# Youssef-Harby/flac-raster

Hardware: AMD Instinct MI355X
Metric: Mpixels/sec encode (create-streaming) + bbox-extract ms, 1/2/4/8 GPU; bit-exact vs ref (higher is better)
Workload: dtype int16; 1 GPU; C4 create-streaming encode (band 1, device-resident); raster=40000x40000x4 int16, tile_size=512, tiles=6241, tiles_rank0=6241, blocksize=4096, compression_level=5, parallelism=single GPU (no exchange), compressed_bytes_rank0=3134407161, compressed_bytes_total=3134407161

## Files before the change

### flac_raster_amd/csrc/frs_encode.hip

```cpp

#include <type_traits>

#include <cstring>
#include <unistd.h>

#include "frs_internal.h"
#include "frs_frame_header.h"
#include "frs_crc16_fold.h"

namespace frs {

template <int DT> struct Elem;
template <> struct Elem<FRS_DT_U8> { using T = uint8_t; static constexpr bool is_float = false; };
template <> struct Elem<FRS_DT_U16> { using T = uint16_t; static constexpr bool is_float = false; };
template <> struct Elem<FRS_DT_I16> { using T = int16_t; static constexpr bool is_float = false; };
template <> struct Elem<FRS_DT_I32> { using T = int32_t; static constexpr bool is_float = false; };
template <> struct Elem<FRS_DT_U32> { using T = uint32_t; static constexpr bool is_float = false; };
template <> struct Elem<FRS_DT_F32> { using T = float; static constexpr bool is_float = true; };
template <> struct Elem<FRS_DT_F64> { using T = double; static constexpr bool is_float = true; };

__device__ inline int64_t f2key(double v) {
    int64_t b = __double_as_longlong(v);
    return b >= 0 ? b : (b ^ 0x7FFFFFFFFFFFFFFFll);
}
// ... 2254 lines not shown
    v ^= bfly_partner<32>(v);
    return uni(v);
}
__device__ inline uint32_t dpp_incl_scan_u32(uint32_t v) {
    v += (uint32_t)__builtin_amdgcn_update_dpp(0, (int)v, 0x111, 0xF, 0xF, false);
    v += (uint32_t)__builtin_amdgcn_update_dpp(0, (int)v, 0x112, 0xF, 0xF, false);
    v += (uint32_t)__builtin_amdgcn_update_dpp(0, (int)v, 0x114, 0xF, 0xF, false);
    v += (uint32_t)__builtin_amdgcn_update_dpp(0, (int)v, 0x118, 0xF, 0xF, false);
    v += (uint32_t)__builtin_amdgcn_update_dpp(0, (int)v, 0x142, 0xA, 0xF, false);
    v += (uint32_t)__builtin_amdgcn_update_dpp(0, (int)v, 0x143, 0xC, 0xF, false);
    return v;
}
__device__ inline uint32_t dpp_wave_shr1(uint32_t v) {
    return (uint32_t)__builtin_amdgcn_update_dpp(0, (int)v, 0x138, 0xF, 0xF, false);
}

typedef short v2s16 __attribute__((ext_vector_type(2)));
__device__ inline int32_t dot2(uint32_t a, uint32_t b, int32_t c) {
    return __builtin_amdgcn_sdot2(__builtin_bit_cast(v2s16, a), __builtin_bit_cast(v2s16, b), c, false);
}
__device__ inline uint32_t pack2(int32_t lo, int32_t hi) { return ((uint32_t)lo & 0xFFFFu) | ((uint32_t)hi << 16); }

__device__ inline int32_t dot2_z(uint32_t a, uint32_t b) {
    int32_t d;
    asm("v_dot2_i32_i16 %0, %1, %2, 0" : "=v"(d) : "v"(a), "v"(b));
    return d;
}

__device__ inline void residual_pair(const uint32_t *E, const uint32_t *C, int shift, int m, int32_t &re, int32_t &ro) {
    const int b = 4 + m;
    const uint32_t o0 = __builtin_amdgcn_perm(E[b], E[b - 1], 0x05040302u);
    const uint32_t o1 = __builtin_amdgcn_perm(E[b - 1], E[b - 2], 0x05040302u);
    const uint32_t o2 = __builtin_amdgcn_perm(E[b - 2], E[b - 3], 0x05040302u);
    const uint32_t o3 = __builtin_amdgcn_perm(E[b - 3], E[b - 4], 0x05040302u);
    int32_t se = dot2_z(E[b - 1], C[0]);
    int32_t so = dot2_z(o0, C[0]);
    se = dot2(E[b - 2], C[1], se);
    so = dot2(o1, C[1], so);
    se = dot2(E[b - 3], C[2], se);
    so = dot2(o2, C[2], so);
    se = dot2(E[b - 4], C[3], se);
    so = dot2(o3, C[3], so);
    const uint32_t v = E[b];
    re = (int32_t)(int16_t)(v & 0xFFFFu) - (se >> shift);
    ro = ((int32_t)v >> 16) - (so >> shift);
}

constexpr uint64_t kFlagAgg = 1ull << 62, kFlagIncl = 2ull << 62, kValMask = (1ull << 62) - 1;


constexpr int kXpowHi = (kXpowBytes + 63) / 64;
constexpr int kBufWordsV3 = kFrameWordsV3 + 64;
constexpr int kSubWords = kFrameWordsV3 + 4;
struct EncV3Shared {
    uint32_t bits[4][kBufWordsV3];
    int16_t lut[kLutCap];
    uint16_t xlo[64];
    uint16_t xhi[kXpowHi + 3];
    uint8_t crc8[256];
    int ticket[2];
    int want[2];
    int lut_tile;
};
static_assert(offsetof(EncV3Shared, lut) + sizeof(int16_t) * kLutCap <= 65536, "LUT beyond 64 KiB of LDS");

struct FbMap {
    uint32_t c, magic, k;
    __device__ inline uint32_t col(uint32_t w) const { return __umul24(w, magic) >> 20; }
    __device__ inline uint32_t operator()(uint32_t w) const {
        return (uint32_t)__mul24((int)col(w), -(int)k) + (w << 6);
    }
};
__device__ inline FbMap fb_map(uint32_t words) {
    const uint32_t c = max(1u, (words + 63) >> 6);
    return FbMap{c, ((1u << 20) + c - 1) / c, 64 * c - 1};
}
__device__ inline void fb_fold(uint32_t *buf, const FbMap &M, int lane) {
    uint32_t *ovr = buf + (M.c << 6) + lane;
    const uint32_t v = *ovr;
    *ovr = 0;
    if (lane < 63 && v) atomicOr(buf + lane + 1, v);
}

__device__ inline void lds_put_bits2(uint32_t *buf, const FbMap &M, uint32_t pos, uint32_t val, int nbits) {
    const uint32_t wi = pos >> 5;
    const uint64_t v = (uint64_t)val << (64 - (int)(pos & 31) - nbits);
    atomicOr(&buf[M(wi)], (uint32_t)(v >> 32));
    atomicOr(&buf[M(wi + 1)], (uint32_t)v);
}

__device__ inline void reg_fence(uint32_t *E) {
#pragma unroll
    for (int m = 0; m < 36; m++) asm volatile("" : "+v"(E[m]));
}

__device__ inline uint32_t sad_u32(uint32_t a, uint32_t b, uint32_t c) {
    uint32_t d;
    asm("v_sad_u32 %0, %1, %2, %3" : "=v"(d) : "v"(a), "v"(b), "v"(c));
    return d;
}

__device__ inline void lds_put_left(uint32_t *buf, const FbMap &M, int nk4, uint32_t pos, uint32_t codeL) {
    const uint32_t hi = __builtin_amdgcn_alignbit(0u, codeL, pos);
    const uint32_t lo = __builtin_amdgcn_alignbit(codeL, 0u, pos);
    const uint32_t wi = pos >> 5;
    uint32_t *p = reinterpret_cast<uint32_t *>(reinterpret_cast<char *>(buf) + (wi << 8) +
                                               __mul24((int)M.col(wi), nk4));
    atomicOr(p, hi);
    atomicOr(p + 64, lo);
}

__device__ inline void lut_gather_pairs(const uint32_t *w, const int16_t *lut, int32_t imin, uint32_t *out) {
    const uint32_t lb = (uint32_t)reinterpret_cast<uintptr_t>(lut);
    const uint32_t c16 = (lb - 2u * (uint32_t)imin) & 0xFFFFu, cc = c16 | (c16 << 16), two = 0x00020002u;
    const char *lds0 = reinterpret_cast<const char *>(lut) - lb;
#pragma unroll
    for (int m = 0; m < 32; m++) {
        uint32_t a;
        asm("v_pk_mad_u16 %0, %1, %2, %3" : "=v"(a) : "v"(w[m]), "v"(two), "v"(cc));
        const uint32_t lo = *reinterpret_cast<const uint16_t *>(lds0 + (a & 0xFFFFu));
        const uint32_t hi = *reinterpret_cast<const uint16_t *>(lds0 + (a >> 16));
        out[m] = lo | (hi << 16);
    }
}

__device__ inline uint32_t zigzag(int32_t r) { return ((uint32_t)r << 1) ^ (uint32_t)(r >> 31); }

struct PendingFrame {
    int64_t f = -1;
    uint64_t fbytes = 0;
    bool ok = true;
    FbMap map{1, 1u << 20, 63};
};

__device__ __forceinline__ void resolve_and_store(const EncodeParams &P, PendingFrame &pf, uint32_t *fbuf, uint8_t *arena,
                                         int64_t arena_cap, int64_t *frame_off, uint64_t *status, int *err, int lane) {
    const int64_t f = pf.f;
    const uint64_t fbytes = pf.fbytes;
    const bool ok = pf.ok;
    const bool l0 = lane == 0;
    uint64_t prefix = 0;
    if (f > 0) {
        constexpr int kPer = 1;
        int64_t hi = f - 1;
        uint64_t accum = 0;
        long spins = 0;
// ... 2 lines not shown
#pragma unroll
            for (int i = 0; i < kPer; i++) {
                const int64_t j = hi - (int64_t)(lane * kPer + i);
                sv[i] = kFlagIncl;
                if (j >= 0) sv[i] = __hip_atomic_load(&status[j], __ATOMIC_RELAXED, __HIP_MEMORY_SCOPE_AGENT);
            }
            int my_first = kPer;
#pragma unroll
            for (int i = kPer - 1; i >= 0; i--)
                if ((sv[i] >> 62) == 2) my_first = i;
            const uint64_t has = __ballot(my_first < kPer);
            const int fl = has ? __builtin_ctzll(has) : 64;
            const int first_i = fl < 64 ? __builtin_amdgcn_readlane(my_first, fl) : kPer;
            bool missing = false;
            uint64_t mine = 0;
#pragma unroll
            for (int i = 0; i < kPer; i++) {
                const bool need = lane < fl || (lane == fl && i <= first_i);
                if (need) {
                    missing |= (sv[i] >> 62) == 0;
                    mine += sv[i] & kValMask;
                }
            }
            if (__ballot(missing)) {
                if (++spins > (1l << 22)) {
                    if (l0) atomicOr(err, 8);
                    break;
                }
                __builtin_amdgcn_s_setprio(0);
                if (spins < 4) __builtin_amdgcn_s_sleep(2);
                else if (spins < 16) __builtin_amdgcn_s_sleep(8);
                else __builtin_amdgcn_s_sleep(32);
                __builtin_amdgcn_s_setprio(2);
                continue;
            }
            accum += dpp_wave_sum_u64(mine);
            if (fl < 64) break;
            hi -= 64 * kPer;
        }
        prefix = accum;
    }
    if (l0) {
        if (f > 0)
            __hip_atomic_store(&status[f], kFlagIncl | (prefix + fbytes), __ATOMIC_RELAXED, __HIP_MEMORY_SCOPE_AGENT);
        frame_off[f] = (int64_t)prefix;
    }
    const FbMap M = pf.map;
    if ((int64_t)(prefix + fbytes) > arena_cap) {
        if (l0) atomicOr(err, 16);
    } else if (fbytes) {
        uint8_t *dst = arena + prefix;
        const uint32_t a0 = min((uint32_t)fbytes, (uint32_t)((16 - (reinterpret_cast<uintptr_t>(dst) & 15)) & 15));
        auto byte_at = [&](uint32_t b) -> uint8_t { return (uint8_t)(fbuf[M(b >> 2)] >> (24 - 8 * (b & 3))); };
        if ((uint32_t)lane < a0) dst[lane] = byte_at((uint32_t)lane);
        const uint32_t n16 = ((uint32_t)fbytes - a0) >> 4;
        const uint32_t r = a0 & 3, sb = a0 >> 2;
        uint4 *d16 = reinterpret_cast<uint4 *>(dst + a0);
        auto chunk = [&](uint32_t ci) {
            const uint32_t wq = sb + 4 * ci;
            const uint32_t w0 = __builtin_bswap32(fbuf[M(wq)]), w1 = __builtin_bswap32(fbuf[M(wq + 1)]);
            const uint32_t w2 = __builtin_bswap32(fbuf[M(wq + 2)]), w3 = __builtin_bswap32(fbuf[M(wq + 3)]);
            const uint32_t w4 = __builtin_bswap32(fbuf[M(wq + 4)]);
            uint4 o4;
            o4.x = __builtin_amdgcn_alignbyte(w1, w0, r);
            o4.y = __builtin_amdgcn_alignbyte(w2, w1, r);
            o4.z = __builtin_amdgcn_alignbyte(w3, w2, r);
            o4.w = __builtin_amdgcn_alignbyte(w4, w3, r);
            d16[ci] = o4;
        };
        const uint32_t c0 = (uint32_t)lane * M.c, c1 = c0 + M.c;
        const uint32_t ci0 = c0 > sb ? (c0 - sb + 3) >> 2 : 0u, ci1 = c1 > sb ? min(n16, (c1 - sb + 3) >> 2) : 0u;
        if (ci0 < ci1) {
            const uint32_t *cp = fbuf + M(sb + 4 * ci0);
            for (uint32_t ci = ci0; ci + 1 < ci1; ci++, cp += 256) {
                const uint32_t w0 = __builtin_bswap32(cp[0]), w1 = __builtin_bswap32(cp[64]);
                const uint32_t w2 = __builtin_bswap32(cp[128]), w3 = __builtin_bswap32(cp[192]);
                const uint32_t w4 = __builtin_bswap32(cp[256]);
                uint4 o4;
                o4.x = __builtin_amdgcn_alignbyte(w1, w0, r);
                o4.y = __builtin_amdgcn_alignbyte(w2, w1, r);
                o4.z = __builtin_amdgcn_alignbyte(w3, w2, r);
                o4.w = __builtin_amdgcn_alignbyte(w4, w3, r);
                d16[ci] = o4;
            }
            chunk(ci1 - 1);
        }
        const uint32_t tb = a0 + 16 * n16 + (uint32_t)lane;
        if (tb < (uint32_t)fbytes) dst[tb] = byte_at(tb);
    }
    if (ok) {
        for (uint32_t i = 0; i < M.c; i++) fbuf[(i << 6) | (uint32_t)lane] = 0;
    } else {
        for (uint32_t i = (uint32_t)lane; i < (uint32_t)kBufWordsV3; i += 64) fbuf[i] = 0;
    }
    pf.f = -1;
}

__device__ inline void fixed_lane_totals(const uint32_t *E, bool l0, uint32_t *tk, uint32_t *hk) {
    constexpr uint32_t M = 0x80000000u;
    const int32_t h1 = (int32_t)E[3] >> 16, h2 = (int16_t)(E[3] & 0xFFFFu);
    const int32_t h3 = (int32_t)E[2] >> 16, h4 = (int16_t)(E[2] & 0xFFFFu);
    uint32_t p0 = (uint32_t)h1 ^ M, p1 = (uint32_t)(h1 - h2) ^ M, p2 = (uint32_t)((h1 - h2) - (h2 - h3)) ^ M;
    uint32_t p3 = (uint32_t)(((h1 - h2) - (h2 - h3)) - ((h2 - h3) - (h3 - h4))) ^ M;
    uint32_t t0 = 0, t1 = 0, t2 = 0, t3 = 0, t4 = 0;
#pragma unroll
    for (int k = 0; k < 5; k++) hk[k] = 0;
#pragma unroll
// ... 252 lines not shown
            bb[c] = best_bits;
            bp[c] = 5 - best_i;
            bk[c] = (int)((Kp[c] >> (4 * best_i)) & 15u);
        }
    };
    auto rice = [&](uint32_t lane_sum, int order, uint32_t &best_bits, int &best_po, int &my_k) {
        if (__ballot(lane_sum >= (1u << 24)) == 0) {
            const uint32_t sm[1] = {lane_sum};
            const int od[1] = {order};
            uint32_t b1[1];
            int p1[1], k1[1];
            rice32m(std::integral_constant<int, 1>{}, sm, od, b1, p1, k1);
            best_bits = b1[0], best_po = p1[0], my_k = k1[0];
        } else {
            rice64(lane_sum, order, best_bits, best_po, my_k);
        }
    };
    rb_f = rb_l = 0;
    po_f = po_l = k_f = k_l = 0;
    if (cand_fixed && cand_lpc && __ballot(sf >= (1u << 24) || sl >= (1u << 24)) == 0) {
        uint32_t bb[2];
        int bp[2], bk[2];
        const uint32_t sm[2] = {sf, sl};
        const int od[2] = {of, ol};
        rice32m(std::integral_constant<int, 2>{}, sm, od, bb, bp, bk);
        rb_f = bb[0], po_f = bp[0], k_f = bk[0];
        rb_l = bb[1], po_l = bp[1], k_l = bk[1];
    } else {
        if (cand_fixed) rice(sf, of, rb_f, po_f, k_f);
        if (cand_lpc) rice(sl, ol, rb_l, po_l, k_l);
    }
}

constexpr int kPrivRows = 34;
constexpr uint32_t kPrivBits = kPrivRows * 32;
static_assert(kBufWordsV3 >= (kPrivRows + 1) * 64, "private rows + the spill row");
static_assert(kBufWordsV3 % 4 == 0, "b128 zeroing");

__device__ inline void zero_wave_buf(uint32_t *buf, int lane) {
    uint4 *b4 = reinterpret_cast<uint4 *>(buf);
#pragma unroll
    for (int i = 0; i < (kBufWordsV3 / 4 + 63) / 64; i++) {
        const int c = lane + 64 * i;
        if (i < kBufWordsV3 / 256 || c < kBufWordsV3 / 4) b4[c] = make_uint4(0u, 0u, 0u, 0u);
    }
}

constexpr int kCrcRows = kFrameWordsV3 / 64;
constexpr int kCrcBias = 192;
static_assert(kFrameWordsV3 % 64 == 0 && kCrcRows <= frs::kCrcFoldSpan && kCrcBias % 64 == 0 && kCrcBias >= 4 * kCrcRows,
              "column CRC");
static_assert(kCrcRows * 64 <= kBufWordsV3 && sizeof(g_xpow_hi) == sizeof(uint16_t) * (kXpowHi + 3),
              "the rows read (in groups of 8, below kCrcRows) are the buffer's; the factor table");
__device__ __forceinline__ uint32_t crc16_cols(const uint32_t *fbuf, const FbMap &M, uint32_t body, const EncV3Shared &S,
                                               int lane) {
    const uint32_t c = frs::crc16_column<kCrcRows, 8>(fbuf + lane, 64, (int)M.c);
    const int m = max(0, (int)body + (kCrcBias - 4 * kCrcRows) - 4 * (int)M.c * lane);
    return dpp_wave_xor_u32(gf_mulmod(gf_mulmod(c, S.xlo[m & 63]), S.xhi[m >> 6]));
}

template <int DT, bool SUB = false, bool ST = false, bool WIDE = false>
__device__ __forceinline__ void encode_frame_v4(const typename Elem<DT>::T *raster, const EncodeParams &P,
                                                const TileGeom *__restrict__ tiles,
                                                const TileNorm *__restrict__ norms,
                                                const SubAnalysis *__restrict__ ana, uint8_t *arena, int64_t arena_cap,
                                                int64_t *frame_off, uint64_t *status, int *err, EncV3Shared &S,
                                                int want, int64_t f, int lane, const int32_t *ftile,
                                                PendingFrame &prev, const uint4 *hdr_tab, int hdr_n,
                                                const uint32_t *pslots, const int64_t *pbytes, int chn = 0,
                                                uint32_t *sub_slots = nullptr, int32_t *sub_bits = nullptr,
                                                int32_t *sub_est = nullptr) {
    using T = typename Elem<DT>::T;
    using Lane = std::conditional_t<WIDE, LaneWide, LanePairs>;
    uint32_t *fbuf = S.bits[uni_if<!WIDE>(threadIdx.x >> 6)];
    const int t = ftile[f];
    const TileGeom g = tiles[t];
    const bool l0 = lane == 0;
    if (!SUB && g.partial && f - g.frame_base == g.nframes - 1) {
        const int64_t si = g.partial - 1;
        const uint64_t nb = (uint64_t)pbytes[si];
        const uint32_t words = (uint32_t)((nb + 3) >> 2);
        const bool ok = words + 2 <= (uint32_t)kFrameWordsV3;
        if (!ok && l0) atomicOr(err, 2);
        const uint64_t fbytes = ok ? nb : 0;
        const FbMap M = fb_map(words + 1);
        __builtin_amdgcn_s_setprio(2);
        if (l0)
            __hip_atomic_store(&status[f], (f == 0 ? kFlagIncl : kFlagAgg) | fbytes, __ATOMIC_RELAXED,
                               __HIP_MEMORY_SCOPE_AGENT);
        if (prev.f >= 0) resolve_and_store(P, prev, fbuf, arena, arena_cap, frame_off, status, err, lane);
        if (ok) {
            const uint32_t *src = pslots + (size_t)si * P.slot_words;
            for (uint32_t w = (uint32_t)lane; w < words; w += 64) fbuf[M(w)] = __builtin_bswap32(src[w]);
        }
        __builtin_amdgcn_s_waitcnt(0xC07F);
        __builtin_amdgcn_wave_barrier();
        __builtin_amdgcn_s_setprio(0);
        prev.f = f, prev.fbytes = fbytes, prev.ok = ok, prev.map = M;
        return;
    }
    TileNorm tn = norms[t];
    if (t != want && tn.mode == kNormLut) tn.mode = kNormSlow;
    const int16_t *lut = S.lut;
    __builtin_amdgcn_s_setprio(2);
    const int64_t fk = f - g.frame_base;
    const int64_t s0 = fk * kMaxBlock;
    constexpr int n = kMaxBlock;
    const int64_t sub = SUB ? f * P.nvch + chn : f;
    const SubAnalysis A = ana[sub];
    const int w = A.wasted;
    const int sbps = 16 - w + ((ST && chn == 3) ? 1 : 0);
    const T *base = raster + (int64_t)(P.band0 + ((ST && chn >= 2) ? 0 : chn)) * P.band_stride + g.r0 * P.row_stride +
                    g.c0;

    auto load_lane = [&](Lane &Ls) __attribute__((always_inline)) {
        Chunk64<DT> ch;
        const uint32_t sl0 = (uint32_t)s0 + 64u * (uint32_t)lane;
        const uint32_t row = udiv_inv(sl0, (uint32_t)g.w, 1.0 / (double)g.w);
        const int col = (int)(sl0 - row * (uint32_t)g.w), vec = (g.w % 64) == 0 ? P.vec_ok : 0;
// ... 334 lines not shown
        const int typecode = type == 0 ? 0 : type == 1 ? 1 : type == 2 ? 8 + of : 32 + ol - 1;
        lds_put_bits2(fbuf, M, hdr_bits, (uint32_t)(typecode << 1) | (w ? 1u : 0u), 8);
        if (w) lds_put_bits2(fbuf, M, hdr_bits + 8 + (uint32_t)(w - 1), 1, 1);
        if (type == 0) lds_put_bits2(fbuf, M, pos0, xi & ((1u << sbps) - 1u), sbps);
        if (type >= 2) {
            uint32_t qq = pos0 + (uint32_t)o * sbps;
            if (type == 3) {
                lds_put_bits2(fbuf, M, qq, (uint32_t)(A.lpc_prec - 1), 4);
                lds_put_bits2(fbuf, M, qq + 4, (uint32_t)lshift & 31u, 5);
                qq += 9 + (uint32_t)o * A.lpc_prec;
            }
            lds_put_bits2(fbuf, M, qq, (uint32_t)po, 6);
        }
    }
    if (type >= 2) {
        const int i = lane & 7;
        const int32_t qi = ana[sub].q[i];
        const bool warm = lane < 8 && i < o, coef = type == 3 && lane >= 8 && lane < 16 && i < o;
        if (warm) lds_put_bits2(fbuf, M, pos0 + (uint32_t)i * sbps, xi & ((1u << sbps) - 1u), sbps);
        if (coef)
            lds_put_bits2(fbuf, M, pos0 + (uint32_t)o * sbps + 9 + (uint32_t)i * A.lpc_prec,
                          (uint32_t)qi & ((1u << A.lpc_prec) - 1u), A.lpc_prec);
    }
    __builtin_amdgcn_s_waitcnt(0xC07F);
    __builtin_amdgcn_wave_barrier();
    if (fold) {
        fb_fold(fbuf, M, lane);
        __builtin_amdgcn_s_waitcnt(0xC07F);
        __builtin_amdgcn_wave_barrier();
    }
    if constexpr (SUB) {
        if (ok) {
            uint32_t *dst = sub_slots + (size_t)sub * kSubWords;
            const uint32_t nw = (end_bits + 31) >> 5;
            for (uint32_t wi = (uint32_t)lane; wi < nw; wi += 64) dst[wi] = fbuf[M(wi)];
            for (uint32_t i = 0; i < M.c; i++) fbuf[(i << 6) | (uint32_t)lane] = 0;
        } else {
            zero_wave_buf(fbuf, lane);
        }
        if (l0) sub_bits[sub] = ok ? (int32_t)end_bits : -1;
        if (l0 && sub_est) sub_est[sub] = (int32_t)best;
        (void)fbytes;
        return;
    }
    if (ok) {
        const uint32_t crc = crc16_cols(fbuf, M, body, S, lane);
        if (l0) lds_put_bits2(fbuf, M, body << 3, crc, 16);
        __builtin_amdgcn_s_waitcnt(0xC07F);
        __builtin_amdgcn_wave_barrier();
    }
    prev.f = f, prev.fbytes = fbytes, prev.ok = ok, prev.map = M;
}

template <int DT, bool SUB = false, bool ST = false, bool WIDE = false>
__global__ void __launch_bounds__(256, sizeof(typename Elem<DT>::T) <= 2 ? (ST ? 2 : 3) : 1) k_encode_v4(const typename Elem<DT>::T *raster, EncodeParams P,
                                                  const TileGeom *__restrict__ tiles,
                                                  const TileNorm *__restrict__ norms, const int16_t *__restrict__ luts,
                                                  const SubAnalysis *__restrict__ ana, uint8_t *arena, int64_t arena_cap,
                                                  int64_t *frame_off, uint64_t *status, int *ticket_ctr, int *err,
                                                  const int32_t *__restrict__ ftile, const uint4 *__restrict__ hdr_tab,
                                                  int hdr_n, const uint32_t *__restrict__ pslots,
                                                  const int64_t *__restrict__ pbytes, uint32_t *sub_slots = nullptr,
                                                  int32_t *sub_bits = nullptr, int32_t *sub_est = nullptr) {
    __shared__ __attribute__((aligned(16))) EncV3Shared S;
    constexpr bool kUni = !WIDE;
    const int wave = (int)uni_if<kUni>(threadIdx.x >> 6), lane = threadIdx.x & 63;
    for (int i = threadIdx.x; i < 256; i += blockDim.x) S.crc8[i] = c_crc8[i];
    for (int i = threadIdx.x; i < 64; i += blockDim.x) S.xlo[i] = g_xpow_bytes[i];
    for (int i = threadIdx.x; i < kXpowHi + 3; i += blockDim.x) S.xhi[i] = g_xpow_hi[i];
    for (int i = threadIdx.x; i < 4 * kBufWordsV3; i += blockDim.x) (&S.bits[0][0])[i] = 0;
    if (threadIdx.x == 0) S.lut_tile = -1;
    PendingFrame prev;
    uint32_t *fbuf = S.bits[wave];
    int it = 0;
    while (true) {
        const int sl = it & 1;
        it++;
        constexpr int kUpfSt = WIDE ? 1 : 3;
        const int upf = ST ? kUpfSt : P.nch;
        const int64_t nunits = SUB ? P.nframes * upf : P.nframes;
        if (threadIdx.x == 0) {
            const int tk = atomicAdd(ticket_ctr, 1);
            S.ticket[sl] = tk;
            const int64_t u0 = (int64_t)tk * 4;
            S.want[sl] = (u0 < nunits) ? ftile[SUB ? u0 / upf : u0] : -1;
        }
        __syncthreads();
        const int64_t fbase = (int64_t)(int)uni_if<kUni>((uint32_t)S.ticket[sl]) * 4;
        if (fbase >= nunits) break;
        const int want = (int)uni_if<kUni>((uint32_t)S.want[sl]);
        if (want != (int)uni_if<kUni>((uint32_t)S.lut_tile)) {
            const TileNorm tw = norms[want];
            if (tw.mode == kNormLut) {
                const int64_t R = min(tw.imax - tw.imin, (int64_t)kLutCap - 1);
                const int16_t *src = luts + (int64_t)want * kLutCap;
                for (int64_t d = threadIdx.x; d <= R; d += blockDim.x) S.lut[d] = src[d];
            }
            __syncthreads();
            if (threadIdx.x == 0) S.lut_tile = want;
        }
        if constexpr (SUB) {
            const int64_t v = fbase + wave;
            if (v < nunits) {
                const int64_t f = v / upf;
                const int chn = WIDE ? 3 : (int)(v - f * upf);
                const TileGeom g = tiles[ftile[f]];
                if (!(g.partial && f - g.frame_base == g.nframes - 1))
                    encode_frame_v4<DT, true, ST, WIDE>(raster, P, tiles, norms, ana, arena, arena_cap, frame_off,
                                                        status, err, S, want, f, lane, ftile, prev, hdr_tab, hdr_n,
                                                        pslots, pbytes, chn, sub_slots, sub_bits, sub_est);
            }
        } else {
            const int64_t f = fbase + wave;
            if (f < nunits)
                encode_frame_v4<DT>(raster, P, tiles, norms, ana, arena, arena_cap, frame_off, status, err, S, want, f,
                                    lane, ftile, prev, hdr_tab, hdr_n, pslots, pbytes);
        }
    }
    if constexpr (!SUB)
        if (prev.f >= 0) resolve_and_store(P, prev, fbuf, arena, arena_cap, frame_off, status, err, lane);
}


__device__ inline int mc_frame_header(uint8_t *h, uint32_t v, int chcode, int sr) {
    return frame_header(h, 4096, sr, 16, chcode, v, c_crc8);
}

__device__ inline int st_pick(const int32_t *est4) {
    const uint32_t e0 = (uint32_t)est4[0], e1 = (uint32_t)est4[1], e2 = (uint32_t)est4[2], e3 = (uint32_t)est4[3];
    const uint32_t bits[4] = {e0 + e1, e0 + e3, e1 + e3, e2 + e3};
    int ca = 0;
    for (int k = 1; k < 4; k++)
        if (bits[k] < bits[ca]) ca = k;
    return ca;
}
__device__ inline void st_subs(int ca, int &a, int &b) {
    a = ca == 2 ? 3 : ca == 3 ? 2 : 0;
    b = ca == 0 ? 1 : ca == 2 ? 1 : 3;
}

__global__ void k_mc_frame_bytes(const EncodeParams P, const TileGeom *tiles, const int32_t *ftile,
                                 const int32_t *sub_bits, const int64_t *pbytes, int64_t *frame_bytes, int *err,
                                 const int32_t *sub_est = nullptr, int8_t *pick = nullptr) {
    const int64_t f = (int64_t)blockIdx.x * blockDim.x + threadIdx.x;
    if (f >= P.nframes) return;
    const TileGeom g = tiles[ftile[f]];
    const int64_t fk = f - g.frame_base;
    if (g.partial && fk == g.nframes - 1) {
        frame_bytes[f] = pbytes[g.partial - 1];
        return;
    }
    uint8_t h[16];
    const bool st = P.nvch == 4 && P.nch == 2;
    int chcode = P.nch - 1, sa = 0, sb = 1;
    if (st) {
        const int ca = st_pick(sub_est + f * 4);
        pick[f] = (int8_t)ca;
        chcode = ca == 0 ? 1 : 7 + ca;
        st_subs(ca, sa, sb);
    }
    int64_t bits = 8 * mc_frame_header(h, (uint32_t)fk, chcode, P.sample_rate);
    for (int c = 0; c < P.nch; c++) {
        const int32_t b = sub_bits[f * P.nvch + (st ? (c ? sb : sa) : c)];
        if (b < 0) atomicOr(err, 2);
        bits += b < 0 ? 0 : b;
    }
    frame_bytes[f] = ((bits + 7) >> 3) + 2;
}

// ... 241 lines not shown
        TileGeom g;
        const int64_t tr = ti / tcols, tc = ti % tcols;
        g.r0 = tr * d->tile_h;
        g.c0 = tc * d->tile_w;
        g.h = (int32_t)std::min<int64_t>(d->tile_h, d->height - g.r0);
        g.w = (int32_t)std::min<int64_t>(d->tile_w, d->width - g.c0);
        const int64_t px = (int64_t)g.h * g.w;
        g.nframes = (int32_t)((px + d->blocksize - 1) / d->blocksize);
        g.frame_base = nframes;
        g.partial = 0;
        nframes += g.nframes;
        tiles.push_back(g);
    }
}

int64_t arena_bound(const frs_encode_desc *d) {
    std::vector<TileGeom> tiles;
    int64_t nframes;
    build_tiles(d, tiles, nframes);
    return nframes * (slot_words_for(d) * 4) + 64;
}

constexpr int kFastDeclined = 1000;

static std::vector<float> tukey_window(int L, float p) {
    std::vector<float> win(L, 1.0f);
    const int Np = (int)(p / 2.0f * (float)L) - 1;
    if (Np > 0)
        for (int k = 0; k <= Np; k++) {
            win[k] = (float)(0.5f - 0.5f * cos(M_PI * k / Np));
            win[L - Np - 1 + k] = (float)(0.5f - 0.5f * cos(M_PI * (k + Np) / Np));
        }
    return win;
}

static int upload_window(frs_ctx *ctx, DevBuf &buf, int L, float p) {
    const std::vector<float> win = tukey_window(L, p);
    FRS_HIP(buf.ensure(sizeof(float) * L));
    FRS_HIP(hipMemcpyAsync(buf.ptr, win.data(), sizeof(float) * L, hipMemcpyHostToDevice, ctx->stream));
    FRS_HIP(hipStreamSynchronize(ctx->stream));
    return FRS_OK;
}

static int align_class(uintptr_t base, std::initializer_list<int> classes, std::initializer_list<int64_t> strides) {
    for (int a : classes) {
        bool ok = base % a == 0;
        for (int64_t s : strides) ok = ok && s % a == 0;
        if (ok) return a;
    }
    return 0;
}

template <typename K, typename... Args>
static int launch_resident(frs_ctx *ctx, K kern, int &nwg_max, int64_t units, Args... args) {
    if (nwg_max == 0) FRS_HIP(hipOccupancyMaxActiveBlocksPerMultiprocessor(&nwg_max, kern, 256, 0));
    int64_t grid = (int64_t)std::max(1, nwg_max) * ctx->num_cus;
    grid = std::min<int64_t>(grid, (units + 3) / 4);
    kern<<<(unsigned)grid, 256, 0, ctx->stream>>>(args...);
    return FRS_OK;
}

enum class EncodePath { Generic, FastMono, FastMulti, FastStereo };

static EncodePath choose_path(const frs_ctx *ctx, const frs_encode_desc *d, const EncodeParams &P, bool is_float,
                              bool allow_fast) {
    const bool eligible = allow_fast && !ctx->force_generic && d->compression_level == 5 && P.bps == 16 &&
                          P.norm_mode == 0 && d->blocksize == 4096 && !is_float;
    if (!eligible) return EncodePath::Generic;
    if (P.nch == 1) return EncodePath::FastMono;
    if (P.nch == 2) return P.nvch == 4 ? EncodePath::FastStereo : EncodePath::Generic;
    return P.nch <= 8 ? EncodePath::FastMulti : EncodePath::Generic;
}

template <int DT> struct EncodeJob {
    using T = typename Elem<DT>::T;
    frs_ctx *ctx;
    const frs_encode_desc *d;
    hipStream_t st;
    EncodeParams P;
    LevelParams lv;
    EncodePath path;
    std::vector<int64_t> key;
    bool geo_hit, dev_tiles;
    std::vector<TileGeom> tiles_local, *tiles;
    int ntiles;
    int64_t nframes, npartial;
    int64_t *hplist;
    size_t pin_wt, pin_res, res_bytes;
    bool stats_vec, fuse_stats;
    const T *raster;
    uint8_t *arena;
    int64_t arena_cap;
    TileGeom *dtiles;
    TileNorm *dnorms;
    SubAnalysis *dana;
    int *err_flag;
    int64_t *tile_off;
    double *tile_min, *tile_max;
    bool stereo_fast() const { return path == EncodePath::FastStereo; }
};

template <int DT>
static int plan_encode(EncodeJob<DT> &J, const void *raster_dev, bool allow_fast) {
    using T = typename Elem<DT>::T;
    frs_ctx *ctx = J.ctx;
    const frs_encode_desc *d = J.d;
    J.key = {d->height, d->width, d->tile_h, d->tile_w, d->tile_begin, d->tile_end, d->blocksize, d->nbands, d->dtype,
             d->bits_per_sample, d->norm_mode, (allow_fast && !ctx->force_generic) ? 1 : 0, d->compression_level};
    J.geo_hit = !ctx->geo.key.empty() && ctx->geo.key == J.key;
    J.tiles = J.geo_hit ? &ctx->geo.tiles : &J.tiles_local;
    J.nframes = ctx->geo.nframes;
// ... 231 lines not shown
    if (const int rc = place()) return rc;
    k_gather_tile_off<<<(ntiles + 1 + 255) / 256, 256, 0, st>>>(dfoff, J.dtiles, ntiles, total,
                                                               ctx->tile_sizes.as<int64_t>());
    std::vector<TileNorm> hn(ntiles);
    FRS_HIP(hipMemcpyAsync(J.tile_off, ctx->tile_sizes.ptr, sizeof(int64_t) * (ntiles + 1), hipMemcpyDeviceToHost, st));
    FRS_HIP(hipMemcpyAsync(hn.data(), J.dnorms, sizeof(TileNorm) * ntiles, hipMemcpyDeviceToHost, st));
    FRS_HIP(hipStreamSynchronize(st));
    prof_collect(ctx);
    for (int t = 0; t < ntiles; t++) {
        J.tile_min[t] = hn[t].dmin;
        J.tile_max[t] = hn[t].dmax;
    }
    return FRS_OK;
}

constexpr int kHdrTabMax = 1 << 16;
static int ensure_header_table(frs_ctx *ctx, const std::vector<TileGeom> &tiles, int sample_rate, int &hdr_n) {
    int32_t maxf = 0;
    for (const TileGeom &tg : tiles) maxf = std::max(maxf, tg.nframes);
    hdr_n = std::min<int32_t>(maxf, kHdrTabMax);
    if (ctx->hdr_tab_n == hdr_n && ctx->hdr_tab_sr == sample_rate) return FRS_OK;
    std::vector<uint32_t> tab((size_t)hdr_n * 4, 0);
    for (int fk = 0; fk < hdr_n; fk++) {
        uint8_t h[16] = {0};
        const int hb = frame_header(h, 4096, sample_rate, 16, 0, (uint32_t)fk, host_crc8());
        uint32_t *row = &tab[(size_t)fk * 4];
        for (int w = 0; w < 4; w++)
            row[w] = ((uint32_t)h[4 * w] << 24) | ((uint32_t)h[4 * w + 1] << 16) | ((uint32_t)h[4 * w + 2] << 8) | h[4 * w + 3];
        row[3] = (row[3] & 0xFFFFFF00u) | (uint32_t)hb;
    }
    FRS_HIP(ctx->hdr_tab.ensure(sizeof(uint32_t) * tab.size() + 16));
    FRS_HIP(hipMemcpyAsync(ctx->hdr_tab.ptr, tab.data(), sizeof(uint32_t) * tab.size(), hipMemcpyHostToDevice,
                           ctx->stream));
    FRS_HIP(hipStreamSynchronize(ctx->stream));
    ctx->hdr_tab_n = hdr_n;
    ctx->hdr_tab_sr = sample_rate;
    return FRS_OK;
}

template <int DT>
static int encode_fast_mono(EncodeJob<DT> &J, int64_t *dpbytes) {
    frs_ctx *ctx = J.ctx;
    hipStream_t st = J.st;
    const int ntiles = J.ntiles;
    const int64_t nframes = J.nframes;
    uint64_t *dstatus = ctx->status.as<uint64_t>();
    int *ticket = reinterpret_cast<int *>(dstatus + nframes);
    FRS_HIP(hipMemsetAsync(dstatus, 0, sizeof(uint64_t) * (nframes + 1) + 64, st));
    int hdr_n = 0;
    if (const int rc = ensure_header_table(ctx, *J.tiles, J.d->sample_rate, hdr_n)) return rc;
    hipEvent_t ev;
    static int nwg_max = 0;
    prof_begin(ctx, "encode", &ev);
    if (const int rc = launch_resident(ctx, k_encode_v4<DT>, nwg_max, nframes, J.raster, J.P, J.dtiles, J.dnorms,
                                       ctx->luts.as<int16_t>(), J.dana, J.arena, J.arena_cap,
                                       ctx->frame_off.as<int64_t>(), dstatus, ticket, J.err_flag,
                                       ctx->frame_tile.as<int32_t>(), ctx->hdr_tab.as<uint4>(), hdr_n,
                                       ctx->slots.as<uint32_t>(), dpbytes, nullptr, nullptr, nullptr))
        return rc;
    prof_end(ctx, "encode", ev);
    FRS_HIP(ctx->host_pack.ensure(J.res_bytes));
    int64_t *dpack = ctx->host_pack.as<int64_t>();
    k_fast_finish<<<(ntiles + 1 + 255) / 256, 256, 0, st>>>(ctx->frame_off.as<int64_t>(), dstatus, J.dtiles, J.dnorms,
                                                           J.err_flag, ntiles, nframes, dpack);
    const int64_t *hpack = ctx->pin.at<int64_t>(J.pin_res);
    FRS_HIP(hipMemcpyAsync(ctx->pin.at<int64_t>(J.pin_res), dpack, J.res_bytes, hipMemcpyDeviceToHost, st));
    FRS_HIP(hipStreamSynchronize(st));
    prof_collect(ctx);
    memcpy(J.tile_off, hpack, sizeof(int64_t) * (ntiles + 1));
    const double *mm = reinterpret_cast<const double *>(hpack + ntiles + 1);
    for (int t = 0; t < ntiles; t++) {
        J.tile_min[t] = mm[2 * t];
        J.tile_max[t] = mm[2 * t + 1];
    }
    const int errv = (int)hpack[3 * (int64_t)ntiles + 1];
    if (errv & 16) {
        ctx->err = "arena too small";
        return FRS_E_NOSPACE;
    }
    if (errv) {
        ctx->err = "fast encode declined, flags " + std::to_string(errv);
        return kFastDeclined;
    }
    return FRS_OK;
}

template <int DT>
static int encode_fast_multi(EncodeJob<DT> &J, int64_t *dpbytes) {
    frs_ctx *ctx = J.ctx;
    const EncodeParams &P = J.P;
    hipStream_t st = J.st;
    const int64_t nframes = J.nframes;
    const bool st2 = J.stereo_fast();
    uint64_t *dstatus = ctx->status.as<uint64_t>();
    int *ticket = reinterpret_cast<int *>(dstatus + nframes);
    const int64_t nsub = nframes * P.nvch;
    FRS_HIP(ctx->sub_slots.ensure(sizeof(uint32_t) * (size_t)nsub * kSubWords));
    FRS_HIP(ctx->sub_bits.ensure(sizeof(int32_t) * (size_t)nsub));
    FRS_HIP(ctx->mc_bytes.ensure(sizeof(int64_t) * (size_t)(nframes + 1)));
    FRS_HIP(hipMemsetAsync(ticket, 0, 2 * sizeof(int), st));
    uint32_t *dsub = ctx->sub_slots.as<uint32_t>();
    int32_t *dsbits = ctx->sub_bits.as<int32_t>();
    int64_t *dmcb = ctx->mc_bytes.as<int64_t>();
    int32_t *dsest = nullptr;
    int8_t *dpick = nullptr;
    if (st2) {
        FRS_HIP(ctx->sub_est.ensure(sizeof(int32_t) * (size_t)nsub));
        FRS_HIP(ctx->st_pick.ensure((size_t)nframes + 64));
        dsest = ctx->sub_est.as<int32_t>();
        dpick = ctx->st_pick.as<int8_t>();
    }
    const int32_t *dftile = ctx->frame_tile.as<int32_t>();
    hipEvent_t ev;
    prof_begin(ctx, "encode", &ev);
    auto launch = [&](auto kern, int &nwg_max, int64_t units, int *tk) {
        return launch_resident(ctx, kern, nwg_max, units, J.raster, P, J.dtiles, J.dnorms, ctx->luts.as<int16_t>(),
                               J.dana, J.arena, J.arena_cap, ctx->frame_off.as<int64_t>(), dstatus, tk, J.err_flag,
                               dftile, ctx->hdr_tab.as<uint4>(), 0, ctx->slots.as<uint32_t>(), dpbytes, dsub, dsbits,
                               dsest);
    };
    if (st2) {
        static int nwg_lrm = 0, nwg_side = 0;
        if (const int rc = launch(k_encode_v4<DT, true, true, false>, nwg_lrm, nframes * 3, ticket)) return rc;
        if (const int rc = launch(k_encode_v4<DT, true, true, true>, nwg_side, nframes, ticket + 1)) return rc;
    } else {
        static int nwg_mc = 0;
        if (const int rc = launch(k_encode_v4<DT, true>, nwg_mc, nsub, ticket)) return rc;
    }
    k_mc_frame_bytes<<<(unsigned)((nframes + 255) / 256), 256, 0, st>>>(P, J.dtiles, dftile, dsbits, dpbytes, dmcb,
                                                                       J.err_flag, dsest, dpick);
    prof_end(ctx, "encode", ev);
    return place_and_report(J, dmcb, kFastDeclined, "fast encode declined, flags ", [&]() -> int {
        const size_t mc_lds = sizeof(uint32_t) * (size_t)(P.nch * kFrameWordsV3 + 16);
        FRS_HIP(hipFuncSetAttribute(reinterpret_cast<const void *>(&k_mc_assemble),
                                    hipFuncAttributeMaxDynamicSharedMemorySize, (int)mc_lds));
        prof_begin(ctx, "assemble", &ev);
        k_mc_assemble<<<(unsigned)nframes, 256, mc_lds, st>>>(P, J.dtiles, dftile, dsub, dsbits,
                                                              ctx->slots.as<uint32_t>(), dpbytes,
                                                              ctx->frame_off.as<int64_t>(), J.arena, dpick);
        prof_end(ctx, "assemble", ev);
        return FRS_OK;
    });
}

template <int DT, bool WIDE, bool ST>
static void launch_generic_analysis(EncodeJob<DT> &J, const EncodeParams &Pa, LpcCand *dcand, const uint8_t *zero) {
    frs_ctx *ctx = J.ctx;
    const unsigned agrid = (unsigned)((J.nframes * J.P.nvch + 127) / 128);
    k_analyze<DT, WIDE, ST><<<agrid, 128, 0, J.st>>>(J.raster, Pa, J.dtiles, J.dnorms, ctx->window.as<float>(), J.dana,
                                                      nullptr, 0, zero);
    if constexpr (WIDE) k_analyze_fixed_wide<DT, ST><<<agrid, 128, 0, J.st>>>(J.raster, Pa, J.dtiles, J.dnorms, J.dana, zero);
    if (dcand)
        k_analyze_lpc_hi<DT, WIDE, ST><<<agrid, 128, 0, J.st>>>(J.raster, J.P, J.dtiles, J.dnorms,
                                                                 ctx->window_hi.as<float>(), J.dana, dcand, J.lv.parts);
}

template <int DT>
static int encode_generic(EncodeJob<DT> &J, const void *raster_dev) {
    using T = typename Elem<DT>::T;
    frs_ctx *ctx = J.ctx;
    const frs_encode_desc *d = J.d;
    const EncodeParams &P = J.P;
    hipStream_t st = J.st;
    const int64_t nframes = J.nframes;
    FRS_HIP(ctx->slots.ensure((size_t)nframes * P.slot_words * 4));
    const int64_t nsub = nframes * P.nvch;
    const bool stereo = P.nvch == 4 && P.nch == 2;
    const bool wide = P.bps > 16;
    EncodeParams Pa = P;
    LpcCand *dcand = nullptr;
// ... 120 lines not shown
```

Baseline: 345,100 Mpixels/s.

## Use 8-wave work-groups for the non-sub int16 encode kernel

Templates the shared-memory struct and encode kernel on the wave count, moving the per-wave bit buffers to the end of the struct. For element types of 2 bytes or less on the non-sub path, each work-group now runs 8 waves that share one LUT load and ticket, with a launch bound for 4 such groups per CU. The launcher checks occupancy against the design target and fails if fewer groups fit. The goal is to spread LUT loads and ticket synchronisation over more frames, at the cost of more LDS per group, more register pressure, and an extra failure path.

```diff
diff --git a/flac_raster_amd/csrc/frs_encode.hip b/flac_raster_amd/csrc/frs_encode.hip
--- a/flac_raster_amd/csrc/frs_encode.hip
+++ b/flac_raster_amd/csrc/frs_encode.hip
@@ -2330,8 +2330,8 @@
 constexpr int kXpowHi = (kXpowBytes + 63) / 64;
 constexpr int kBufWordsV3 = kFrameWordsV3 + 64;
 constexpr int kSubWords = kFrameWordsV3 + 4;
+template <int NW = 4>
 struct EncV3Shared {
-    uint32_t bits[4][kBufWordsV3];
     int16_t lut[kLutCap];
     uint16_t xlo[64];
     uint16_t xhi[kXpowHi + 3];
@@ -2339,8 +2339,10 @@
     int ticket[2];
     int want[2];
     int lut_tile;
+    alignas(16) uint32_t bits[NW][kBufWordsV3];
 };
-static_assert(offsetof(EncV3Shared, lut) + sizeof(int16_t) * kLutCap <= 65536, "LUT beyond 64 KiB of LDS");
+static_assert(offsetof(EncV3Shared<8>, lut) + sizeof(int16_t) * kLutCap <= 65536, "LUT beyond 64 KiB of LDS");
+static_assert(sizeof(EncV3Shared<8>) <= 81920, "two 8-wave work-groups per CU");
 
 struct FbMap {
     uint32_t c, magic, k;
@@ -2370,6 +2372,11 @@
 __device__ inline void reg_fence(uint32_t *E) {
 #pragma unroll
     for (int m = 0; m < 36; m++) asm volatile("" : "+v"(E[m]));
+}
+
+__device__ inline uint32_t local_u32(uint32_t v) {
+    asm volatile("" : "+v"(v));
+    return v;
 }
 
 __device__ inline uint32_t sad_u32(uint32_t a, uint32_t b, uint32_t c) {
@@ -2478,7 +2485,7 @@
         uint8_t *dst = arena + prefix;
         const uint32_t a0 = min((uint32_t)fbytes, (uint32_t)((16 - (reinterpret_cast<uintptr_t>(dst) & 15)) & 15));
         auto byte_at = [&](uint32_t b) -> uint8_t { return (uint8_t)(fbuf[M(b >> 2)] >> (24 - 8 * (b & 3))); };
-        if ((uint32_t)lane < a0) dst[lane] = byte_at((uint32_t)lane);
+        if ((uint32_t)lane < a0) dst[lane] = byte_at(local_u32((uint32_t)lane));
         const uint32_t n16 = ((uint32_t)fbytes - a0) >> 4;
         const uint32_t r = a0 & 3, sb = a0 >> 2;
         uint4 *d16 = reinterpret_cast<uint4 *>(dst + a0);
@@ -2837,19 +2844,20 @@
               "column CRC");
 static_assert(kCrcRows * 64 <= kBufWordsV3 && sizeof(g_xpow_hi) == sizeof(uint16_t) * (kXpowHi + 3),
               "the rows read (in groups of 8, below kCrcRows) are the buffer's; the factor table");
-__device__ __forceinline__ uint32_t crc16_cols(const uint32_t *fbuf, const FbMap &M, uint32_t body, const EncV3Shared &S,
+template <class Shared>
+__device__ __forceinline__ uint32_t crc16_cols(const uint32_t *fbuf, const FbMap &M, uint32_t body, const Shared &S,
                                                int lane) {
     const uint32_t c = frs::crc16_column<kCrcRows, 8>(fbuf + lane, 64, (int)M.c);
     const int m = max(0, (int)body + (kCrcBias - 4 * kCrcRows) - 4 * (int)M.c * lane);
     return dpp_wave_xor_u32(gf_mulmod(gf_mulmod(c, S.xlo[m & 63]), S.xhi[m >> 6]));
 }
 
-template <int DT, bool SUB = false, bool ST = false, bool WIDE = false>
+template <int DT, bool SUB = false, bool ST = false, bool WIDE = false, int NW = 4>
 __device__ __forceinline__ void encode_frame_v4(const typename Elem<DT>::T *raster, const EncodeParams &P,
                                                 const TileGeom *__restrict__ tiles,
                                                 const TileNorm *__restrict__ norms,
                                                 const SubAnalysis *__restrict__ ana, uint8_t *arena, int64_t arena_cap,
-                                                int64_t *frame_off, uint64_t *status, int *err, EncV3Shared &S,
+                                                int64_t *frame_off, uint64_t *status, int *err, EncV3Shared<NW> &S,
                                                 int want, int64_t f, int lane, const int32_t *ftile,
                                                 PendingFrame &prev, const uint4 *hdr_tab, int hdr_n,
                                                 const uint32_t *pslots, const int64_t *pbytes, int chn = 0,
@@ -3290,8 +3298,9 @@
     prev.f = f, prev.fbytes = fbytes, prev.ok = ok, prev.map = M;
 }
 
-template <int DT, bool SUB = false, bool ST = false, bool WIDE = false>
-__global__ void __launch_bounds__(256, sizeof(typename Elem<DT>::T) <= 2 ? (ST ? 2 : 3) : 1) k_encode_v4(const typename Elem<DT>::T *raster, EncodeParams P,
+template <int DT, bool SUB> constexpr int enc_nw() { return !SUB && sizeof(typename Elem<DT>::T) <= 2 ? 8 : 4; }
+template <int DT, bool SUB = false, bool ST = false, bool WIDE = false, int NW = 4>
+__global__ void __launch_bounds__(64 * NW, NW == 8 ? 4 : sizeof(typename Elem<DT>::T) <= 2 ? (ST ? 2 : 3) : 1) k_encode_v4(const typename Elem<DT>::T *raster, EncodeParams P,
                                                   const TileGeom *__restrict__ tiles,
                                                   const TileNorm *__restrict__ norms, const int16_t *__restrict__ luts,
                                                   const SubAnalysis *__restrict__ ana, uint8_t *arena, int64_t arena_cap,
@@ -3300,13 +3309,13 @@
                                                   int hdr_n, const uint32_t *__restrict__ pslots,
                                                   const int64_t *__restrict__ pbytes, uint32_t *sub_slots = nullptr,
                                                   int32_t *sub_bits = nullptr, int32_t *sub_est = nullptr) {
-    __shared__ __attribute__((aligned(16))) EncV3Shared S;
+    __shared__ __attribute__((aligned(16))) EncV3Shared<NW> S;
     constexpr bool kUni = !WIDE;
     const int wave = (int)uni_if<kUni>(threadIdx.x >> 6), lane = threadIdx.x & 63;
     for (int i = threadIdx.x; i < 256; i += blockDim.x) S.crc8[i] = c_crc8[i];
     for (int i = threadIdx.x; i < 64; i += blockDim.x) S.xlo[i] = g_xpow_bytes[i];
     for (int i = threadIdx.x; i < kXpowHi + 3; i += blockDim.x) S.xhi[i] = g_xpow_hi[i];
-    for (int i = threadIdx.x; i < 4 * kBufWordsV3; i += blockDim.x) (&S.bits[0][0])[i] = 0;
+    for (int i = threadIdx.x; i < NW * kBufWordsV3; i += blockDim.x) (&S.bits[0][0])[i] = 0;
     if (threadIdx.x == 0) S.lut_tile = -1;
     PendingFrame prev;
     uint32_t *fbuf = S.bits[wave];
@@ -3320,11 +3329,11 @@
         if (threadIdx.x == 0) {
             const int tk = atomicAdd(ticket_ctr, 1);
             S.ticket[sl] = tk;
-            const int64_t u0 = (int64_t)tk * 4;
+            const int64_t u0 = (int64_t)tk * NW;
             S.want[sl] = (u0 < nunits) ? ftile[SUB ? u0 / upf : u0] : -1;
         }
         __syncthreads();
-        const int64_t fbase = (int64_t)(int)uni_if<kUni>((uint32_t)S.ticket[sl]) * 4;
+        const int64_t fbase = (int64_t)(int)uni_if<kUni>((uint32_t)S.ticket[sl]) * NW;
         if (fbase >= nunits) break;
         const int want = (int)uni_if<kUni>((uint32_t)S.want[sl]);
         if (want != (int)uni_if<kUni>((uint32_t)S.lut_tile)) {
@@ -3332,7 +3341,8 @@
             if (tw.mode == kNormLut) {
                 const int64_t R = min(tw.imax - tw.imin, (int64_t)kLutCap - 1);
                 const int16_t *src = luts + (int64_t)want * kLutCap;
-                for (int64_t d = threadIdx.x; d <= R; d += blockDim.x) S.lut[d] = src[d];
+                for (int64_t d = NW == 8 ? local_u32(threadIdx.x) : threadIdx.x; d <= R; d += blockDim.x)
+                    S.lut[d] = src[d];
             }
             __syncthreads();
             if (threadIdx.x == 0) S.lut_tile = want;
@@ -3344,15 +3354,16 @@
                 const int chn = WIDE ? 3 : (int)(v - f * upf);
                 const TileGeom g = tiles[ftile[f]];
                 if (!(g.partial && f - g.frame_base == g.nframes - 1))
-                    encode_frame_v4<DT, true, ST, WIDE>(raster, P, tiles, norms, ana, arena, arena_cap, frame_off,
+                    encode_frame_v4<DT, true, ST, WIDE, NW>(raster, P, tiles, norms, ana, arena, arena_cap, frame_off,
                                                         status, err, S, want, f, lane, ftile, prev, hdr_tab, hdr_n,
                                                         pslots, pbytes, chn, sub_slots, sub_bits, sub_est);
             }
         } else {
             const int64_t f = fbase + wave;
             if (f < nunits)
-                encode_frame_v4<DT>(raster, P, tiles, norms, ana, arena, arena_cap, frame_off, status, err, S, want, f,
-                                    lane, ftile, prev, hdr_tab, hdr_n, pslots, pbytes);
+                encode_frame_v4<DT, false, false, false, NW>(raster, P, tiles, norms, ana, arena, arena_cap, frame_off,
+                                                             status, err, S, want, f, lane, ftile, prev, hdr_tab, hdr_n,
+                                                             pslots, pbytes);
         }
     }
     if constexpr (!SUB)
@@ -3700,11 +3711,17 @@
 }
 
 template <typename K, typename... Args>
-static int launch_resident(frs_ctx *ctx, K kern, int &nwg_max, int64_t units, Args... args) {
-    if (nwg_max == 0) FRS_HIP(hipOccupancyMaxActiveBlocksPerMultiprocessor(&nwg_max, kern, 256, 0));
+static int launch_resident(frs_ctx *ctx, K kern, int &nwg_max, int threads, int per_wg, int need_wg, int64_t units,
+                           Args... args) {
+    if (nwg_max == 0) FRS_HIP(hipOccupancyMaxActiveBlocksPerMultiprocessor(&nwg_max, kern, threads, 0));
+    if (nwg_max < need_wg) {
+        ctx->err = "encoder occupancy: " + std::to_string(nwg_max) + " work-groups of " + std::to_string(threads) +
+                   " threads per CU, built for " + std::to_string(need_wg);
+        return FRS_E_HIP;
+    }
     int64_t grid = (int64_t)std::max(1, nwg_max) * ctx->num_cus;
-    grid = std::min<int64_t>(grid, (units + 3) / 4);
-    kern<<<(unsigned)grid, 256, 0, ctx->stream>>>(args...);
+    grid = std::min<int64_t>(grid, (units + per_wg - 1) / per_wg);
+    kern<<<(unsigned)grid, threads, 0, ctx->stream>>>(args...);
     return FRS_OK;
 }
 
@@ -4042,7 +4059,9 @@
     hipEvent_t ev;
     static int nwg_max = 0;
     prof_begin(ctx, "encode", &ev);
-    if (const int rc = launch_resident(ctx, k_encode_v4<DT>, nwg_max, nframes, J.raster, J.P, J.dtiles, J.dnorms,
+    constexpr int NW = enc_nw<DT, false>();
+    if (const int rc = launch_resident(ctx, k_encode_v4<DT, false, false, false, NW>, nwg_max, 64 * NW, NW,
+                                       NW == 8 ? 2 : 0, nframes, J.raster, J.P, J.dtiles, J.dnorms,
                                        ctx->luts.as<int16_t>(), J.dana, J.arena, J.arena_cap,
                                        ctx->frame_off.as<int64_t>(), dstatus, ticket, J.err_flag,
                                        ctx->frame_tile.as<int32_t>(), ctx->hdr_tab.as<uint4>(), hdr_n,
@@ -4104,8 +4123,8 @@
     hipEvent_t ev;
     prof_begin(ctx, "encode", &ev);
     auto launch = [&](auto kern, int &nwg_max, int64_t units, int *tk) {
-        return launch_resident(ctx, kern, nwg_max, units, J.raster, P, J.dtiles, J.dnorms, ctx->luts.as<int16_t>(),
-                               J.dana, J.arena, J.arena_cap, ctx->frame_off.as<int64_t>(), dstatus, tk, J.err_flag,
+        return launch_resident(ctx, kern, nwg_max, 256, 4, 0, units, J.raster, P, J.dtiles, J.dnorms,
+                               ctx->luts.as<int16_t>(), J.dana, J.arena, J.arena_cap, ctx->frame_off.as<int64_t>(), dstatus, tk, J.err_flag,
                                dftile, ctx->hdr_tab.as<uint4>(), 0, ctx->slots.as<uint32_t>(), dpbytes, dsub, dsbits,
                                dsest);
     };
```

New measurement: 351,400 Mpixels/s, median of 6. +1.8%, better.
